# Luoyadan/CRB-active-3Ddet

Hardware: AMD Instinct MI355X
Metric: frames/s SECOND fwd+bwd, KITTI 20k-pt clouds (higher is better)
Workload: dtype f32

## Files before the change

### crb-active-3ddet_amd/crbhip/bnrelu.py

```python
import torch

from ._lib import lib, check, ptr, cur_stream, require_cuda


FUSE_RUNNING = __import__('os').environ.get('CRB_BN_FUSE_RUNNING', '1') == '1'
TICKETS = __import__('os').environ.get('CRB_BN_TICKETS', '1') == '1'
_ticket_areas = {}


def _scratch(dev, wsb):
    ws = torch.empty((wsb,), dtype=torch.uint8, device=dev)
    if not TICKETS:
        return ws, None
    key = (dev.index, torch.cuda.current_stream(dev).cuda_stream)
    t = _ticket_areas.get(key)
    if t is None:
        t = _ticket_areas[key] = torch.zeros((lib.crb_bn_ticket_ints(),), dtype=torch.int32, device=dev)
    return ws, t


def _bn_check(rc, what):
    if rc != 0:
        _ticket_areas.clear()
    check(rc, what)
# ... 216 lines not shown
@torch.no_grad()
def bn_apply_(x, bn, relu=True):
    require_cuda(x)
    n, C = x.shape
    assert x.is_contiguous()
    invstd = _invstd(bn)
    check(lib.crb_bn_relu_apply(ptr(x), n, C, ptr(bn.running_mean.contiguous()), ptr(invstd), ptr(bn.weight.contiguous()),
                                ptr(bn.bias.contiguous()), int(relu), ptr(x), 0, cur_stream(x.device)), 'crb_bn_relu_apply')
    return x


@torch.no_grad()
def bn_apply_into(x, bn, relu, out, col):
    import ctypes
    require_cuda(x, out)
    n, C = x.shape
    assert x.is_contiguous() and out.is_contiguous() and out.shape[0] == n and col + C <= out.shape[1]
    invstd = _invstd(bn)
    check(lib.crb_bn_relu_apply(ptr(x), n, C, ptr(bn.running_mean.contiguous()), ptr(invstd), ptr(bn.weight.contiguous()),
                                ptr(bn.bias.contiguous()), int(relu), ctypes.c_void_p(out.data_ptr() + 4 * col),
                                out.shape[1], cur_stream(x.device)), 'crb_bn_relu_apply')
    return out


class _BNReLUConcatTrain(torch.autograd.Function):

    @staticmethod
    def forward(ctx, relu, *args):
        import ctypes
        k = len(args) // 7
        xs = [args[7 * i].contiguous() for i in range(k)]
        n, dev = xs[0].shape[0], xs[0].device
        widths = [x.shape[1] for x in xs]
        total = sum(widths)
        out = torch.empty((n, total), dtype=torch.float32, device=dev)
        saved, col = [], 0
        for i, x in enumerate(xs):
            gamma, beta, eps, rm, rv, mom = args[7 * i + 1:7 * i + 7]
            C = widths[i]
            mean = torch.empty((C,), dtype=torch.float32, device=dev)
            var, invstd = torch.empty_like(mean), torch.empty_like(mean)
            wsb = lib.crb_bn_workspace_bytes(n, C)
            ws, tk = _scratch(dev, wsb)
            g, b = gamma.contiguous().float(), beta.contiguous().float()
            zptr = ctypes.c_void_p(out.data_ptr() + 4 * col)
            _bn_check(lib.crb_bn_relu_forward(ptr(x), n, C, ptr(g), ptr(b), float(eps), int(relu), zptr, total, ptr(mean),
                                          ptr(var), ptr(invstd), ptr(rm), ptr(rv), None, float(mom), ptr(ws), wsb, ptr(tk),
                                          cur_stream(dev)), 'crb_bn_relu_forward')
            _touch(rm, rv)
            saved += [x, mean, invstd, g, b]
            col += C
        ctx.save_for_backward(*saved)
        ctx.relu, ctx.widths = int(relu), widths
        return out

    @staticmethod
    def backward(ctx, dz):
        import ctypes
        dz = dz.contiguous().float()
        n, total = dz.shape
        saved = ctx.saved_tensors
        grads, col = [None], 0
        for i, C in enumerate(ctx.widths):
            x, mean, invstd, g, b = saved[5 * i:5 * i + 5]
            dev = x.device
            dx = torch.empty_like(x)
            dgamma = torch.empty((C,), dtype=torch.float32, device=dev)
            dbeta = torch.empty_like(dgamma)
            wsb = lib.crb_bn_workspace_bytes(n, C)
            ws, tk = _scratch(dev, wsb)
            dzp = ctypes.c_void_p(dz.data_ptr() + 4 * col)
            _bn_check(lib.crb_bn_relu_backward(ptr(x), dzp, total, n, C, ptr(mean), ptr(invstd), ptr(g), ptr(b), ctx.relu,
                                           ptr(dx), ptr(dgamma), ptr(dbeta), ptr(ws), wsb, ptr(tk), cur_stream(dev)),
                  'crb_bn_relu_backward')
            grads += [dx, dgamma, dbeta, None, None, None, None]
            col += C
        return tuple(grads)


def bn_relu_concat(xs, bns, relu=True):
    if _GROUPS is not None and _GROUPS.G > 1:
        off = _GROUPS.offsets(xs[0])
        if not torch.is_grad_enabled():
            total = sum(x.shape[1] for x in xs)
            out = torch.empty((xs[0].shape[0], total), dtype=torch.float32, device=xs[0].device)
            col = 0
            for x, bn in zip(xs, bns):
                _frames_forward(x, off, bn, relu, out, col)
                col += x.shape[1]
            return out
        with frame_groups(1):
            return torch.cat([bn_relu_concat([x[a:b] for x in xs], bns, relu) for a, b in zip(off[:-1], off[1:])], 0)
    args = []
    for x, bn in zip(xs, bns):
        with torch.no_grad():
            bn.num_batches_tracked += 1
        args += [x, bn.weight, bn.bias, bn.eps, bn.running_mean, bn.running_var, float(bn.momentum)]
    return _BNReLUConcatTrain.apply(relu, *args)


class _BNReLUMaxConcatTrain(torch.autograd.Function):

    @staticmethod
    def forward(ctx, *args):
        import ctypes
        k = len(args) // 8
        xs = [args[8 * i].contiguous() for i in range(k)]
        nss = [int(args[8 * i + 1]) for i in range(k)]
        dev = xs[0].device
        M = xs[0].shape[0] // nss[0]
        widths = [x.shape[1] for x in xs]
        total = sum(widths)
        out = torch.empty((M, total), dtype=torch.float32, device=dev)
        saved, col = [], 0
        for i, x in enumerate(xs):
            gamma, beta, eps, rm, rv, mom = args[8 * i + 2:8 * i + 8]
            C, ns = widths[i], nss[i]
            assert x.shape[0] == M * ns
            mean = torch.empty((C,), dtype=torch.float32, device=dev)
            var, invstd = torch.empty_like(mean), torch.empty_like(mean)
            arg = torch.empty((M, C), dtype=torch.int32, device=dev)
            wsb = lib.crb_bn_workspace_bytes(M * ns, C)
            ws, tk = _scratch(dev, wsb)
            g, b = gamma.contiguous().float(), beta.contiguous().float()
            zptr = ctypes.c_void_p(out.data_ptr() + 4 * col)
            _bn_check(lib.crb_bn_relu_max_forward(ptr(x), M, ns, C, ptr(g), ptr(b), float(eps), zptr, total, ptr(arg),
                                              ptr(mean), ptr(var), ptr(invstd), ptr(rm), ptr(rv), None, float(mom), ptr(ws), wsb,
                                              ptr(tk), cur_stream(dev)), 'crb_bn_relu_max_forward')
            _touch(rm, rv)
            saved += [x, mean, invstd, g, b, arg]
            col += C
        ctx.save_for_backward(*saved)
        ctx.widths, ctx.nss = widths, nss
        return out

    @staticmethod
    def backward(ctx, gz):
        import ctypes
        gz = gz.contiguous().float()
        M, total = gz.shape
        saved = ctx.saved_tensors
        grads, col = [], 0
        for i, (C, ns) in enumerate(zip(ctx.widths, ctx.nss)):
            x, mean, invstd, g, b, arg = saved[6 * i:6 * i + 6]
            dev = x.device
            dx = torch.empty_like(x)
            dgamma = torch.empty((C,), dtype=torch.float32, device=dev)
            dbeta = torch.empty_like(dgamma)
            wsb = lib.crb_bn_workspace_bytes(M * ns, C)
            ws, tk = _scratch(dev, wsb)
            gp = ctypes.c_void_p(gz.data_ptr() + 4 * col)
# ... 46 lines not shown
```

### crb-active-3ddet_amd/pcdet/models/backbones_2d/base_bev_backbone.py

```python
import numpy as np
import torch
import torch.nn as nn

from crbhip import bnrelu

from ...utils.fold_utils import fold_conv_bn
from ...utils.linear_rows import LinearRows, rows_view, rows_to_nchw


ROWS_TRAIN = True
ROWS_GEMM = True
WINOGRAD = __import__('os').environ.get('CRB_WINOGRAD', '1') != '0'


def _wino_fold(w, shift):
    from crbhip import winograd
    return winograd.weights_forward2(w), shift.contiguous()


def _wino_ok(conv, x, pad=None):
    if not WINOGRAD or not isinstance(conv, nn.Conv2d) or not x.is_cuda or x.dtype != torch.float32:
        return False
    from crbhip import winograd
    p = tuple(conv.padding) if pad is None else tuple(pad)
# ... 189 lines not shown
    def forward(self, data_dict):
        spatial_features = data_dict['spatial_features']
        ups = []
        x = spatial_features
        if not self.training and not torch.is_grad_enabled():
            cat_ok = x.is_cuda and x.is_contiguous(memory_format=torch.channels_last) and self._can_fuse_concat_eval(x)
            pre = []
            for i, blk in enumerate(self.blocks):
                x = self._run_folded(blk, x)
                if cat_ok:
                    pre.append(self._up(self.deblocks[i][0], x))
                else:
                    ups.append(self._run_folded(self.deblocks[i], x) if len(self.deblocks) > 0 else x)
            if cat_ok and all(p.is_contiguous(memory_format=torch.channels_last) and p.shape[2:] == pre[0].shape[2:]
                              for p in pre):
                n, _, h, w_ = pre[0].shape
                cat = torch.empty((n * h * w_, sum(p.shape[1] for p in pre)), dtype=torch.float32, device=x.device)
                col = 0
                for d, p in zip(self.deblocks, pre):
                    bnrelu.bn_apply_into(p.permute(0, 2, 3, 1).reshape(n * h * w_, p.shape[1]), d[1], True, cat, col)
                    col += p.shape[1]
                ups = [cat.view(n, h, w_, cat.shape[1]).permute(0, 3, 1, 2)]
            elif cat_ok:
                ups = [self._run_folded(nn.Sequential(*list(d)[1:]), p) for d, p in zip(self.deblocks, pre)]
            x = torch.cat(ups, dim=1) if len(ups) > 1 else ups[0]
            if len(self.deblocks) > len(self.blocks):
                x = self._run_folded(self.deblocks[-1], x)
            data_dict['spatial_features_2d'] = x
            return data_dict
        run = self._run_rows_train if (ROWS_TRAIN and x.is_cuda and x.is_contiguous(memory_format=torch.channels_last)) \
            else (lambda seq, t: seq(t))
        if run == self._run_rows_train and torch.is_grad_enabled():
            from crbhip import winograd
            if winograd.PREPARE:
                winograd.prepare_weights2([m.weight for blk in self.blocks for m in blk
                                           if isinstance(m, nn.Conv2d) and m.kernel_size == (3, 3) and m.stride == (1, 1)
                                           and m.weight.is_cuda])
        fuse_cat = ROWS_TRAIN and x.is_cuda and self._can_fuse_concat(x)
        pre = []
        for i, blk in enumerate(self.blocks):
            x = run(blk, x)
            stride = int(spatial_features.shape[2] / x.shape[2])
            data_dict['spatial_features_%dx' % stride] = x
            if fuse_cat:
                pre.append(self._up(self.deblocks[i][0], x))
            else:
                ups.append(run(self.deblocks[i], x) if len(self.deblocks) > 0 else x)
        if fuse_cat and all(p.is_contiguous(memory_format=torch.channels_last) and p.shape[2:] == pre[0].shape[2:]
                            for p in pre):
            n, _, h, w_ = pre[0].shape
            rows = [p.permute(0, 2, 3, 1).reshape(n * h * w_, p.shape[1]) for p in pre]
            cat = bnrelu.bn_relu_concat(rows, [d[1] for d in self.deblocks[:len(pre)]], relu=True)
            ups = [cat.view(n, h, w_, cat.shape[1]).permute(0, 3, 1, 2)]
        elif fuse_cat:
            ups = [d[2](d[1](p)) for d, p in zip(self.deblocks, pre)]
        x = torch.cat(ups, dim=1) if len(ups) > 1 else ups[0]
        if len(self.deblocks) > len(self.blocks):
            x = self.deblocks[-1](x)
        data_dict['spatial_features_2d'] = x
        if x.is_cuda:
            from crbhip import winograd
            winograd.forget_prepared_forward()
        return data_dict
```

### crb-active-3ddet_amd/pcdet/models/dense_heads/anchor_head_single.py

```python
import numpy as np
import torch
import torch.nn as nn

from ...utils.linear_rows import LinearRows, rows_view
from .anchor_head_template import AnchorHeadTemplate


FUSED_HEAD_CONVS = True
ROWS_GEMM = True


class AnchorHeadSingle(AnchorHeadTemplate):
    def __init__(self, model_cfg, input_channels, num_class, class_names, grid_size, point_cloud_range,
                 predict_boxes_when_training=True, **kwargs):
        super().__init__(model_cfg=model_cfg, num_class=num_class, class_names=class_names, grid_size=grid_size,
                         point_cloud_range=point_cloud_range, predict_boxes_when_training=predict_boxes_when_training)
        self.num_anchors_per_location = sum(self.num_anchors_per_location)
        n = self.num_anchors_per_location
        self.conv_cls = nn.Conv2d(input_channels, n * self.num_class, kernel_size=1)
        self.conv_box = nn.Conv2d(input_channels, n * self.box_coder.code_size, kernel_size=1)
        if self.model_cfg.get('USE_DIRECTION_CLASSIFIER', None) is not None:
            self.conv_dir_cls = nn.Conv2d(input_channels, n * self.model_cfg.NUM_DIR_BINS, kernel_size=1)
        else:
            self.conv_dir_cls = None
        self.lazy_box_decode = False
        self.init_weights()

    def init_weights(self):
        pi = 0.01
        nn.init.constant_(self.conv_cls.bias, -np.log((1 - pi) / pi))
        nn.init.normal_(self.conv_box.weight, mean=0, std=0.001)

    def forward(self, data_dict):
        feats = data_dict['spatial_features_2d']
        if FUSED_HEAD_CONVS:
            heads = [self.conv_cls, self.conv_box] + ([self.conv_dir_cls] if self.conv_dir_cls is not None else [])
            w = torch.cat([h.weight for h in heads], 0)
            b = torch.cat([h.bias for h in heads], 0)
            rows = rows_view(feats) if (ROWS_GEMM and feats.is_cuda) else None
            if rows is not None:
                n, _, h, w_ = feats.shape
                y = LinearRows.apply(rows, w.flatten(1), b).view(n, h, w_, w.shape[0])
            else:
                y = torch.nn.functional.conv2d(feats, w, b).permute(0, 2, 3, 1)
            outs = torch.split(y, [h.out_channels for h in heads], dim=3)
            cls_preds, box_preds = outs[0].contiguous(), outs[1].contiguous()
            dir_cls_preds = outs[2].contiguous() if self.conv_dir_cls is not None else None
        else:
            cls_preds = self.conv_cls(feats).permute(0, 2, 3, 1).contiguous()
            box_preds = self.conv_box(feats).permute(0, 2, 3, 1).contiguous()
            dir_cls_preds = None
            if self.conv_dir_cls is not None:
                dir_cls_preds = self.conv_dir_cls(feats).permute(0, 2, 3, 1).contiguous()
        self.forward_ret_dict['cls_preds'] = cls_preds
        self.forward_ret_dict['box_preds'] = box_preds
        self.forward_ret_dict['dir_cls_preds'] = dir_cls_preds
        if self.training:
            self.forward_ret_dict.update(self.assign_targets(gt_boxes=data_dict['gt_boxes']))
        if not self.training or self.predict_boxes_when_training:
            B = data_dict['batch_size']
            data_dict['rpn_preds'] = cls_preds
            data_dict['cls_preds_normalized'] = False
            if self.lazy_box_decode:
                data_dict['batch_cls_preds'] = cls_preds.view(B, -1, self.num_class).float()
                data_dict['batch_box_decoder'] = lambda idx: self.generate_predicted_boxes(
                    batch_size=B, cls_preds=cls_preds, box_preds=box_preds, dir_cls_preds=dir_cls_preds, anchor_idx=idx)[1]
                data_dict.pop('batch_box_preds', None)
            else:
                batch_cls_preds, batch_box_preds = self.generate_predicted_boxes(
                    batch_size=B, cls_preds=cls_preds, box_preds=box_preds, dir_cls_preds=dir_cls_preds)
                data_dict['batch_cls_preds'] = batch_cls_preds
                data_dict['batch_box_preds'] = batch_box_preds
        return data_dict
```

### include/crb_hip.h

```cpp
#ifndef CRB_HIP_H
#define CRB_HIP_H
#include <stdint.h>

#ifdef __cplusplus
extern "C" {
#endif

#define CRB_OK 0
#define CRB_ERR_ARG (-1)
#define CRB_ERR_WORKSPACE (-2)
#define CRB_ERR_LAUNCH (-3)
#define CRB_ERR_UNSUPPORTED (-4)

int crb_abi_version(void);

int64_t crb_voxelize_workspace_bytes(int64_t n_points, int B, int max_voxels, int max_points);
int crb_voxelize(const float* points, int64_t n_points, int num_features,
                 const int32_t* frame_offsets, int B,
                 const float* range_min_xyz, const float* voxel_size_xyz, const int32_t* grid_xyz,
                 int max_voxels, int max_points,
                 float* voxels, int32_t* coords, int32_t* num_points, float* mean_features,
                 int32_t* num_voxels_out,
                 void* workspace, int64_t workspace_bytes, void* stream);

// ... 385 lines not shown
int64_t crb_winograd2_stats_slabs(int N, int H, int W);
int crb_conv3x3_winograd2_stats_nhwc(const float* x, const float* U, float* y, float* stats, int N, int H, int W, int cin, int cout,
                                     void* stream);

int crb_winograd4_supported(int cin, int cout, int H, int W);
int64_t crb_winograd4_weights_bytes(int cin, int cout);
int crb_winograd4_weights_conv(const float* w, int64_t so, int64_t si, int64_t sky, int64_t skx, void* U, int conv_cin, int conv_cout,
                               int mode, void* stream);
int crb_winograd4_weights_conv_multi(int n, const float* const* w, const int64_t* strides, void* const* U, const int32_t* conv_cin,
                                     const int32_t* conv_cout, const int32_t* mode, void* stream);
int crb_conv3x3_winograd4_nhwc(const float* x, const void* U, float* y, int N, int H, int W, int cin, int cout, const float* bias,
                               int relu, void* stream);
int64_t crb_winograd4_stats_slabs(int N, int H, int W);
int crb_conv3x3_winograd4_stats_nhwc(const float* x, const void* U, float* y, float* stats, int N, int H, int W, int cin, int cout,
                                     void* stream);
int crb_winograd4c_supported(int cin, int cout, int H, int W);
int crb_conv3x3_winograd4c_nhwc(const float* x, const void* U, float* y, int N, int H, int W, int cin, int cout,
                                const float* bias, int relu, void* stream);
int64_t crb_winograd4c_stats_slabs(int N, int H, int W);
int crb_conv3x3_winograd4c_stats_nhwc(const float* x, const void* U, float* y, float* stats, int N, int H, int W, int cin,
                                      int cout, void* stream);

int crb_bev_blocks_geometry(int N, int H, int W, int32_t* geom);
int64_t crb_bev_blocks_ints(int N, int H, int W);
int crb_bev_blocks(const int32_t* indices, int64_t n, int N, int H, int W, int32_t* out, int64_t out_ints, void* stream);
int crb_conv3x3_winograd4c_blocks_nhwc(const float* x, const void* U, float* y, float* stats, int N, int H, int W, int cin,
                                       int cout, const int32_t* list, const int32_t* count, const int32_t* rest,
                                       const int32_t* rest_count, void* stream);

int crb_winograd2_wgrad_supported(int cin, int cout, int H, int W);
int64_t crb_winograd2_wgrad_workspace_bytes(int cin, int cout);
int crb_winograd2_wgrad(const float* x, const float* dy, float* dw, int64_t so, int64_t si, int64_t sky, int64_t skx,
                        int N, int H, int W, int cin, int cout, void* workspace, int64_t workspace_bytes, void* stream);
int crb_winograd4_wgrad_supported(int cin, int cout, int H, int W);
int64_t crb_winograd4_wgrad_workspace_bytes(int cin, int cout);
int crb_winograd4_wgrad(const float* x, const float* dy, float* dw, int64_t so, int64_t si, int64_t sky, int64_t skx,
                        int N, int H, int W, int cin, int cout, void* workspace, int64_t workspace_bytes, void* stream);
int crb_winograd4_wgrad_blocks(const float* x, const float* dy, float* dw, int64_t so, int64_t si, int64_t sky, int64_t skx,
                               int N, int H, int W, int cin, int cout, const int32_t* list, const int32_t* count,
                               void* workspace, int64_t workspace_bytes, void* stream);

int crb_rows_gemm4_supported(int cin, int cout, int stride, int direction);
int64_t crb_rows_gemm4_weights_bytes(int cin, int cout, int stride);
int crb_rows_gemm4_weights(const float* w, int64_t s_ci, int64_t s_co, int64_t s_a, int64_t s_b, void* image, int cin, int cout,
                           int stride, int direction, void* stream);
int crb_rows_gemm4_forward(const float* x, const void* image, float* y, int N, int H, int W, int cin, int cout, int stride,
                           void* stream);
int crb_rows_gemm4_input_grad(const float* dy, const void* image, float* dx, int N, int H, int W, int cin, int cout, int stride,
                              void* stream);
int64_t crb_rows_gemm4_wgrad_workspace_bytes(int cin, int cout, int stride);
int crb_rows_gemm4_wgrad(const float* x, const float* dy, float* dw, int64_t s_ci, int64_t s_co, int64_t s_a, int64_t s_b, int N,
                         int H, int W, int cin, int cout, int stride, void* workspace, int64_t workspace_bytes, void* stream);

int crb_cu_reservation(int cus, void* stream);

int crb_bev_interpolate_forward(const float* bev, int B, int H, int W, int C, const float* keypoints, int64_t M, float x_min,
                                float y_min, float voxel_x, float voxel_y, float bev_stride, float* out, void* stream);
int crb_bev_interpolate_backward(const float* dout, int B, int H, int W, int C, const float* keypoints, int64_t M, float x_min,
                                 float y_min, float voxel_x, float voxel_y, float bev_stride, float* dbev, void* stream);

int crb_roi_bev_pool(const float* bev, int B, int H, int W, int C, const float* rois, int roi_row_stride, int R, int grid_size,
                     double x_min, double y_min, double cell_x, double cell_y, float* out, void* stream);

int crb_voxel_pool_supported(int C, int nsample);
int crb_voxel_query(const float* xyz, int64_t N, const float* new_xyz, const int32_t* new_coords, int64_t M, int B,
                    const int32_t* shape_dhw, const int32_t* ranges_zyx, float radius, int nsample, const int64_t* hkeys,
                    const int32_t* hvals, int64_t capacity, int32_t* idx, int32_t* cnt, void* stream);
int64_t crb_voxel_pool_moments_workspace_bytes(int64_t M);
int crb_voxel_pool_moments(const float* xyz, const float* new_xyz, const int32_t* idx, const int32_t* cnt, int64_t M, int nsample,
                           double* sums, void* workspace, int64_t workspace_bytes, void* stream);
int crb_voxel_pool_forward(const float* features_in, int64_t N, int C, const float* xyz, const float* new_xyz, const int32_t* idx,
                           const int32_t* cnt, int64_t M, int nsample, int pool, const float* A, const float* b, float* out,
                           void* stream);
int64_t crb_voxel_pool_backward_workspace_bytes(int64_t M, int C);
int crb_voxel_pool_backward(const float* grad_out, const float* features_in, int64_t N, int C, const float* xyz,
                            const float* new_xyz, const int32_t* idx, const int32_t* cnt, int64_t M, int nsample, int pool,
                            const float* A, const float* b, float* d_features, float* g_sel, int32_t* a_row, float* d_Ab,
                            void* workspace, int64_t workspace_bytes, void* stream);

int crb_pillar_vfe_supported(int C, int T, int Cout);
int crb_pillar_vfe_num_moments(int C);
int64_t crb_pillar_vfe_moments_workspace_bytes(int64_t M, int C);
int crb_pillar_vfe_moments(const float* voxels, const int32_t* num_points, const int32_t* coords, int64_t M, int T, int C,
                           const float* voxel_size, const float* offsets, double* sums, void* workspace, int64_t workspace_bytes,
                           void* stream);
int crb_pillar_vfe_forward(const float* voxels, const int32_t* num_points, const int32_t* coords, int64_t M, int T, int C,
                           const float* voxel_size, const float* offsets, const float* A, const float* b, int Cout, float* out,
                           void* stream);
int64_t crb_pillar_vfe_backward_workspace_bytes(int64_t M, int C, int Cout);
int crb_pillar_vfe_backward(const float* grad_out, const float* voxels, const int32_t* num_points, const int32_t* coords, int64_t M,
                            int T, int C, const float* voxel_size, const float* offsets, const float* A, const float* b, int Cout,
                            double* d_sums, void* workspace, int64_t workspace_bytes, void* stream);

#define CRB_LOSSNET_MAX_LAYERS 4
typedef struct CrbLossNetArgs {
  const float* x[CRB_LOSSNET_MAX_LAYERS];
  const float* w[CRB_LOSSNET_MAX_LAYERS];
  const float* gamma[CRB_LOSSNET_MAX_LAYERS];
  const float* beta[CRB_LOSSNET_MAX_LAYERS];
  float* running_mean[CRB_LOSSNET_MAX_LAYERS];
  float* running_var[CRB_LOSSNET_MAX_LAYERS];
  int64_t* num_batches_tracked[CRB_LOSSNET_MAX_LAYERS];
  int32_t channels[CRB_LOSSNET_MAX_LAYERS];
  int32_t num_layer;
  int32_t rows_per_frame;
  int32_t frames;
// ... 110 lines not shown
```

Measured before the change: 488.9.

## Fuse head 1x1 conv backward with preceding BN-ReLU concat backward

Adds a fused backward path that joins the anchor head's 1x1 linear layer with the deblock BatchNorm+ReLU concat that feeds it. The head input gradient dz = dy·W is never materialised. A sums kernel uses split-bf16 MFMA to compute the BN reductions and dW directly from x, dy and the saved statistics, and an apply kernel recomputes dz on the fly to produce dx for both branches. This removes the full-size dz tensor, its write and reread, and a separate wgrad GEMM. The cost is a three-way bf16 split to keep f32-like accuracy, and support for only 2 branches of width 128/256 with K of 60 or 72.

```diff
diff --git a/crb-active-3ddet_amd/crbhip/bnrelu.py b/crb-active-3ddet_amd/crbhip/bnrelu.py
--- a/crb-active-3ddet_amd/crbhip/bnrelu.py
+++ b/crb-active-3ddet_amd/crbhip/bnrelu.py
@@ -292,30 +292,47 @@
             col += C
         ctx.save_for_backward(*saved)
         ctx.relu, ctx.widths = int(relu), widths
+        ctx.set_materialize_grads(False)
+        global _CONCAT_SAVED
+        _CONCAT_SAVED = saved
         return out
 
     @staticmethod
     def backward(ctx, dz):
-        import ctypes
+        if dz is None:
+            return (None,) * (1 + 7 * len(ctx.widths))
         dz = dz.contiguous().float()
-        n, total = dz.shape
         saved = ctx.saved_tensors
         grads, col = [None], 0
         for i, C in enumerate(ctx.widths):
             x, mean, invstd, g, b = saved[5 * i:5 * i + 5]
-            dev = x.device
-            dx = torch.empty_like(x)
-            dgamma = torch.empty((C,), dtype=torch.float32, device=dev)
-            dbeta = torch.empty_like(dgamma)
-            wsb = lib.crb_bn_workspace_bytes(n, C)
-            ws, tk = _scratch(dev, wsb)
-            dzp = ctypes.c_void_p(dz.data_ptr() + 4 * col)
-            _bn_check(lib.crb_bn_relu_backward(ptr(x), dzp, total, n, C, ptr(mean), ptr(invstd), ptr(g), ptr(b), ctx.relu,
-                                           ptr(dx), ptr(dgamma), ptr(dbeta), ptr(ws), wsb, ptr(tk), cur_stream(dev)),
-                  'crb_bn_relu_backward')
+            dx, dgamma, dbeta = concat_backward(x, dz, col, mean, invstd, g, b, ctx.relu)
             grads += [dx, dgamma, dbeta, None, None, None, None]
             col += C
         return tuple(grads)
+
+
+_CONCAT_SAVED = None
+
+
+def concat_backward(x, dz, col, mean, invstd, g, b, relu=1, want_dx=True):
+    import ctypes
+    n, C = x.shape
+    dev = x.device
+    dx = torch.empty_like(x) if want_dx else None
+    dgamma = torch.empty((C,), dtype=torch.float32, device=dev)
+    dbeta = torch.empty_like(dgamma)
+    wsb = lib.crb_bn_workspace_bytes(n, C)
+    ws, tk = _scratch(dev, wsb)
+    dzp = ctypes.c_void_p(dz.data_ptr() + 4 * col)
+    _bn_check(lib.crb_bn_relu_backward(ptr(x), dzp, dz.shape[1], n, C, ptr(mean), ptr(invstd), ptr(g), ptr(b), int(relu), ptr(dx),
+                                       ptr(dgamma), ptr(dbeta), ptr(ws), wsb, ptr(tk), cur_stream(dev)), 'crb_bn_relu_backward')
+    return dx, dgamma, dbeta
+
+
+def concat_reduce(x, dz, col, mean, invstd, g, b, relu=1):
+    _, dgamma, dbeta = concat_backward(x, dz, col, mean, invstd, g, b, relu, want_dx=False)
+    return dbeta, dgamma
 
 
 def bn_relu_concat(xs, bns, relu=True):
@@ -336,7 +353,14 @@
         with torch.no_grad():
             bn.num_batches_tracked += 1
         args += [x, bn.weight, bn.bias, bn.eps, bn.running_mean, bn.running_var, float(bn.momentum)]
-    return _BNReLUConcatTrain.apply(relu, *args)
+    global _CONCAT_SAVED
+    out = _BNReLUConcatTrain.apply(relu, *args)
+    saved, _CONCAT_SAVED = _CONCAT_SAVED, None
+    if torch.is_grad_enabled() and saved is not None:
+        from . import head_bn
+        out._crb_head_bn = head_bn.Record(out, [(x, bn.weight, bn.bias) for x, bn in zip(xs, bns)],
+                                          [tuple(saved[5 * i:5 * i + 5]) for i in range(len(xs))], relu)
+    return out
 
 
 class _BNReLUMaxConcatTrain(torch.autograd.Function):
diff --git a/crb-active-3ddet_amd/crbhip/head_bn.py b/crb-active-3ddet_amd/crbhip/head_bn.py
--- /dev/null
+++ b/crb-active-3ddet_amd/crbhip/head_bn.py
@@ -0,0 +1,171 @@
+import os
+
+import torch
+
+from ._lib import lib, check, ptr, cur_stream
+
+ENABLED = os.environ.get('CRB_HEAD_BN', '1') == '1'
+DEFAULT_LAUNCHES = 'sums,apply'
+LAUNCHES = set(v.strip() for v in os.environ.get('CRB_HEAD_BN_LAUNCHES', DEFAULT_LAUNCHES).split(',') if v.strip())
+
+TRACE = None
+
+
+def supported(widths, K):
+    widths = [int(v) for v in widths]
+    return len(widths) > 0 and len(set(widths)) == 1 and bool(lib.crb_head_bn_supported(len(widths), widths[0], int(K)))
+
+
+class Record(object):
+
+    def __init__(self, rows, inputs, saved, relu):
+        self.rows_ptr, self.rows_shape = rows.data_ptr(), tuple(rows.shape)
+        self.inputs = inputs
+        self.saved = saved
+        self.relu = bool(relu)
+
+    @property
+    def widths(self):
+        return [s[0].shape[1] for s in self.saved]
+
+
+def dispatch(rows, record, K):
+    if not ENABLED:
+        return 'vendor', 'CRB_HEAD_BN=0'
+    if record is None:
+        return 'vendor', 'the map carries no BatchNorm record (eval mode, grad mode off, frame_groups or another producer)'
+    if not torch.is_grad_enabled():
+        return 'vendor', 'grad mode is off'
+    if not (rows.is_cuda and rows.dim() == 2 and rows.dtype == torch.float32 and rows.is_contiguous()):
+        return 'vendor', 'the map is not a contiguous f32 device row matrix'
+    if rows.data_ptr() != record.rows_ptr or tuple(rows.shape) != record.rows_shape:
+        return 'vendor', 'the record belongs to another map'
+    if not record.relu:
+        return 'vendor', 'BatchNorm without ReLU'
+    if not supported(record.widths, K):
+        return 'vendor', 'no instance for widths %s with K = %d' % (record.widths, K)
+    return 'fused', ','.join(sorted(LAUNCHES & {'sums', 'apply'}))
+
+
+_WS = {}
+
+
+def _workspace(dev, nbytes):
+    key = (dev, torch.cuda.current_stream(dev).cuda_stream)
+    ws = _WS.get(key)
+    if ws is None or ws.numel() < nbytes:
+        ws = _WS[key] = torch.empty((nbytes,), dtype=torch.uint8, device=dev)
+    return ws
+
+
+def params(saved):
+    return torch.cat([torch.stack([s[1], s[2], s[3], s[4]]) for s in saved], 1).contiguous()
+
+
+def sums(xs, par, dout, K):
+    n, width, nb = xs[0].shape[0], xs[0].shape[1], len(xs)
+    out = torch.empty((int(lib.crb_head_bn_sums_count(nb, width, K)),), dtype=torch.float64, device=dout.device)
+    nbytes = int(lib.crb_head_bn_workspace_bytes(nb, width, K))
+    ws = _workspace(dout.device, nbytes)
+    check(lib.crb_head_bn_sums(ptr(xs[0]), ptr(xs[1]), ptr(par), ptr(dout), n, nb, width, K, ptr(out), ptr(ws), ws.numel(),
+                               cur_stream(dout.device)), 'crb_head_bn_sums')
+    return out
+
+
+def finalize(s, w, par, nb, width, K, want_bias=True):
+    Ct = nb * width
+    dgb = torch.empty((2, Ct), dtype=torch.float32, device=w.device)
+    dw = torch.empty((K, Ct), dtype=torch.float32, device=w.device)
+    db = torch.empty((K,), dtype=torch.float32, device=w.device) if want_bias else None
+    check(lib.crb_head_bn_finalize(ptr(s), ptr(w), ptr(par), nb, width, K, ptr(dgb), ptr(dw), ptr(db), cur_stream(w.device)),
+          'crb_head_bn_finalize')
+    return dgb, dw, db
+
+
+def apply(xs, par, dgb, dout, w, K):
+    n, width, nb = xs[0].shape[0], xs[0].shape[1], len(xs)
+    img = torch.empty((int(lib.crb_head_bn_weights_bytes(nb, width, K)),), dtype=torch.uint8, device=w.device)
+    check(lib.crb_head_bn_weights(ptr(w), ptr(img), nb, width, K, cur_stream(w.device)), 'crb_head_bn_weights')
+    dxs = [torch.empty_like(x) for x in xs]
+    check(lib.crb_head_bn_apply(ptr(xs[0]), ptr(xs[1]), ptr(par), ptr(dgb), ptr(dout), ptr(img), n, nb, width, K, ptr(dxs[0]),
+                                ptr(dxs[1]), cur_stream(w.device)), 'crb_head_bn_apply')
+    return dxs
+
+
+def _note(what):
+    if TRACE is not None:
+        TRACE.append(what)
+
+
+class _HeadBN(torch.autograd.Function):
+
+    @staticmethod
+    def forward(ctx, rows, w, b, record, *branch):
+        ctx.set_materialize_grads(False)
+        ctx.nb = len(record.saved)
+        ctx.launches = set(LAUNCHES)
+        flat = [t for s in record.saved for t in s]
+        ctx.save_for_backward(w, *(flat + ([rows] if 'sums' not in ctx.launches else [])))
+        return torch.addmm(b, rows, w.t())
+
+    @staticmethod
+    def backward(ctx, dy):
+        nb = ctx.nb
+        none = (None,) * (4 + 3 * nb)
+        if dy is None:
+            return none
+        t = ctx.saved_tensors
+        w = t[0].contiguous()
+        saved = [t[1 + 5 * i:6 + 5 * i] for i in range(nb)]
+        xs = [s[0] for s in saved]
+        need = ctx.needs_input_grad
+        need_x = any(need[4 + 3 * i] for i in range(nb))
+        need_gb = any(need[5 + 3 * i] or need[6 + 3 * i] for i in range(nb))
+        dy = dy.contiguous().float()
+        K, width = w.shape[0], xs[0].shape[1]
+        dw = db = dgb = None
+        dxs = [None] * nb
+        dz = None
+        if need[1] or need_gb or need_x:
+            par = params(saved)
+            if 'sums' in ctx.launches:
+                _note('sums')
+                dgb, dw, db = finalize(sums(xs, par, dy, K), w, par, nb, width, K, want_bias=need[2])
+            else:
+                from pcdet.utils.linear_rows import tall_t_matmul
+                from . import bnrelu
+                _note('vendor_sums')
+                dz = dy @ w
+                dgb = torch.empty((2, nb * width), dtype=torch.float32, device=dy.device)
+                for i, (x, mean, invstd, g, be) in enumerate(saved):
+                    dgb[:, i * width:(i + 1) * width] = torch.stack(bnrelu.concat_reduce(x, dz, i * width, mean, invstd, g, be))
+                dw = tall_t_matmul(dy, t[-1]) if need[1] else None
+            if need_x:
+                if 'apply' in ctx.launches:
+                    _note('apply')
+                    dxs = apply(xs, par, dgb, dy, w, K)
+                else:
+                    from . import bnrelu
+                    _note('vendor_apply')
+                    dz = dy @ w if dz is None else dz
+                    dxs = [bnrelu.concat_backward(x, dz, i * width, mean, invstd, g, be)[0]
+                           for i, (x, mean, invstd, g, be) in enumerate(saved)]
+        if need[2] and db is None:
+            db = dy.sum(0)
+        grads = [None, dw if need[1] else None, db if need[2] else None, None]
+        for i in range(nb):
+            sl = slice(i * width, (i + 1) * width)
+            grads += [dxs[i] if need[4 + 3 * i] else None,
+                      dgb[1, sl] if (dgb is not None and need[5 + 3 * i]) else None,
+                      dgb[0, sl] if (dgb is not None and need[6 + 3 * i]) else None]
+        return tuple(grads)
+
+
+def linear(rows, w, b, record):
+    path, _ = dispatch(rows, record, w.shape[0])
+    if path != 'fused':
+        return None
+    if b is None or w.dim() != 2 or w.dtype != torch.float32 or w.shape[1] != rows.shape[1]:
+        return None
+    branch = [t for trio in record.inputs for t in trio]
+    return _HeadBN.apply(rows, w, b, record, *branch)
diff --git a/crb-active-3ddet_amd/csrc/head_bn.hip b/crb-active-3ddet_amd/csrc/head_bn.hip
--- /dev/null
+++ b/crb-active-3ddet_amd/csrc/head_bn.hip
@@ -0,0 +1,472 @@
+#include <atomic>
+#include <type_traits>
+#include <utility>
+#include "crb_common.h"
+#include "winograd_split.h"
+#include "../../include/crb_hip.h"
+
+typedef float hb_f32x4 __attribute__((ext_vector_type(4)));
+typedef float hb_f32x16 __attribute__((ext_vector_type(16)));
+
+namespace {
+
+constexpr int HB_NT = 256;
+constexpr int HB_RBG = 8;
+constexpr int HB_COLP = 96;
+
+template <typename F, int... I>
+__device__ __forceinline__ void hb_static_for_impl(F&& f, std::integer_sequence<int, I...>) {
+  (f(std::integral_constant<int, I>{}), ...);
+}
+template <int N, typename F>
+__device__ __forceinline__ void hb_static_for(F&& f) { hb_static_for_impl(f, std::make_integer_sequence<int, N>{}); }
+
+__device__ constexpr int hb_pass_a(int p) { return p == 0 ? 0 : p == 1 ? 2 : p == 2 ? 1 : p == 3 ? 0 : p == 4 ? 1 : 0; }
+__device__ constexpr int hb_pass_b(int p) { return p == 0 ? 2 : p == 1 ? 0 : p == 2 ? 1 : p == 3 ? 1 : 0; }
+
+__device__ __forceinline__ hb_f32x16 hb_mfma(const bf16x8& a, const bf16x8& b, const hb_f32x16& c) {
+  return __builtin_amdgcn_mfma_f32_32x32x16_bf16(a, b, c, 0, 0, 0);
+}
+
+struct HbSplit8 {
+  float sv[2], s1[2], s2[2];
+  u32x4 q0, q1, q2;
+  template <int E>
+  __device__ __forceinline__ void put(float v) {
+    constexpr int hh = E & 1;
+    sv[hh] = v;
+    split3f(v, s1[hh], s2[hh]);
+    if constexpr (hh == 1) {
+      q0[E >> 1] = __builtin_amdgcn_perm(__float_as_uint(sv[1]), __float_as_uint(sv[0]), 0x07060302u);
+      q1[E >> 1] = __builtin_amdgcn_perm(__float_as_uint(s1[1]), __float_as_uint(s1[0]), 0x07060302u);
+      q2[E >> 1] = __builtin_amdgcn_perm(__float_as_uint(s2[1]), __float_as_uint(s2[0]), 0x07060302u);
+    }
+  }
+  __device__ __forceinline__ void get(bf16x8 (&f)[3]) const {
+    f[0] = __builtin_bit_cast(bf16x8, q0);
+    f[1] = __builtin_bit_cast(bf16x8, q1);
+    f[2] = __builtin_bit_cast(bf16x8, q2);
+  }
+};
+
+struct HsArgs {
+  const float* x0;
+  const float* x1;
+  const float* par;
+  const float* dout;
+  float* part;
+  double* colpart;
+  int64_t n;
+  int C, Ct, K, ncg;
+  int nchunks, nranges;
+};
+
+template <int NKB>
+__global__ __launch_bounds__(HB_NT, 2) void head_bn_sums_kernel(HsArgs a) {
+  const int lane = threadIdx.x & 63, wave = __builtin_amdgcn_readfirstlane(threadIdx.x >> 6);
+  const int r = lane & 31, h = lane >> 5;
+  const int cg = blockIdx.x % a.ncg, range = blockIdx.x / a.ncg;
+  const int cb = cg * 4 + wave, c = cb * 32 + r;
+  const int branch = (cb * 32) / a.C;
+  const float* const xbase = branch ? a.x1 : a.x0;
+  const unsigned cl = (unsigned)(c - branch * a.C);
+  const float mu = a.par[c], is = a.par[a.Ct + c], ga = a.par[2 * a.Ct + c], be = a.par[3 * a.Ct + c];
+  const int c_first = (int)((int64_t)range * a.nchunks / a.nranges);
+  const int c_end = (int)((int64_t)(range + 1) * a.nchunks / a.nranges);
+  const bool do_col = cg == 0 && wave == 0;
+
+  hb_f32x16 s2[NKB], s3[NKB];
+  double colsum[NKB];
+  bool kin[NKB];
+  unsigned kc[NKB];
+#pragma unroll
+  for (int kb = 0; kb < NKB; ++kb) {
+#pragma unroll
+    for (int i = 0; i < 16; ++i) { s2[kb][i] = 0.f; s3[kb][i] = 0.f; }
+    colsum[kb] = 0.0;
+    kin[kb] = 32 * kb + r < a.K;
+    kc[kb] = (unsigned)(kin[kb] ? 32 * kb + r : a.K - 1);
+  }
+
+  auto load = [&](int q, float (&xv)[8], float (&dv)[NKB][8]) __attribute__((always_inline)) {
+    const int64_t r0 = (int64_t)q * 16, rem = a.n - r0;
+    const unsigned last = (unsigned)(rem < 16 ? rem : 16) - 1u;
+    const float* const xq = xbase + r0 * a.C;
+    const float* const dq = a.dout + r0 * a.K;
+#pragma unroll
+    for (int j = 0; j < 8; ++j) {
+      const unsigned rj = min((unsigned)(8 * h + j), last);
+      xv[j] = xq[rj * (unsigned)a.C + cl];
+#pragma unroll
+      for (int kb = 0; kb < NKB; ++kb) dv[kb][j] = dq[rj * (unsigned)a.K + kc[kb]];
+    }
+  };
+
+  float xv[8], dv[NKB][8];
+  if (c_first < c_end) load(c_first, xv, dv);
+  for (int q = c_first; q < c_end; ++q) {
+    float xn[8], dn[NKB][8];
+    load(q + 1 < c_end ? q + 1 : q, xn, dn);
+    const int64_t left64 = a.n - ((int64_t)q * 16 + 8 * h);
+    const int left = left64 < 8 ? (int)left64 : 8;
+
+    HbSplit8 sx;
+    u32x4 mk;
+    unsigned mlo = 0;
+    hb_static_for<8>([&](auto jc) __attribute__((always_inline)) {
+      constexpr int j = decltype(jc)::value;
+      const float xh = (xv[j] - mu) * is;
+      const float z = ga * xh + be;
+      const bool m = j < left && z > 0.f;
+      sx.put<j>(m ? xh : 0.f);
+      const unsigned mb = m ? 0x3f80u : 0u;
+      if constexpr (j & 1) mk[j >> 1] = mlo | (mb << 16);
+      else mlo = mb;
+    });
+    bf16x8 X[3];
+    sx.get(X);
+    const bf16x8 Mk = __builtin_bit_cast(bf16x8, mk);
+
+    hb_static_for<NKB>([&](auto kc_) __attribute__((always_inline)) {
+      constexpr int kb = decltype(kc_)::value;
+      HbSplit8 sd;
+      float d[8];
+      hb_static_for<8>([&](auto jc) __attribute__((always_inline)) {
+        constexpr int j = decltype(jc)::value;
+        d[j] = (j < left && kin[kb]) ? dv[kb][j] : 0.f;
+        sd.put<j>(d[j]);
+      });
+      if (do_col) {
+#pragma unroll
+        for (int j = 0; j < 8; ++j) colsum[kb] += (double)d[j];
+      }
+      bf16x8 D[3];
+      sd.get(D);
+      hb_f32x16 t2, t3;
+#pragma unroll
+      for (int i = 0; i < 16; ++i) { t2[i] = 0.f; t3[i] = 0.f; }
+      t2 = hb_mfma(D[2], Mk, t2);
+      t2 = hb_mfma(D[1], Mk, t2);
+      t2 = hb_mfma(D[0], Mk, t2);
+      hb_static_for<6>([&](auto pc) __attribute__((always_inline)) {
+        constexpr int p = decltype(pc)::value;
+        t3 = hb_mfma(D[hb_pass_a(p)], X[hb_pass_b(p)], t3);
+      });
+      s2[kb] += t2;
+      s3[kb] += t3;
+    });
+#pragma unroll
+    for (int j = 0; j < 8; ++j) {
+      xv[j] = xn[j];
+#pragma unroll
+      for (int kb = 0; kb < NKB; ++kb) dv[kb][j] = dn[kb][j];
+    }
+  }
+
+  float* const p2 = a.part + ((int64_t)range * 2) * a.K * a.Ct + c;
+  float* const p3 = p2 + (int64_t)a.K * a.Ct;
+  hb_static_for<NKB>([&](auto kc_) __attribute__((always_inline)) {
+    constexpr int kb = decltype(kc_)::value;
+    hb_static_for<16>([&](auto ic) __attribute__((always_inline)) {
+      constexpr int i = decltype(ic)::value;
+      const int k = 32 * kb + (i & 3) + 8 * (i >> 2) + 4 * h;
+      if (k < a.K) {
+        p2[(int64_t)k * a.Ct] = s2[kb][i];
+        p3[(int64_t)k * a.Ct] = s3[kb][i];
+      }
+    });
+    if (do_col) a.colpart[((int64_t)range * 2 + h) * HB_COLP + 32 * kb + r] = colsum[kb];
+  });
+}
+
+__global__ __launch_bounds__(256) void head_bn_reduce_kernel(const float* __restrict__ part, const double* __restrict__ colpart,
+                                                             int nranges, int K, int Ct, double* __restrict__ sums) {
+  __shared__ double sh[8][32];
+  const int64_t per = (int64_t)2 * K * Ct;
+  const int il = threadIdx.x & 31, sl = threadIdx.x >> 5;
+  const int64_t id = (int64_t)blockIdx.x * 32 + il;
+  double s = 0.0;
+  if (id < per) {
+    for (int g = sl; g < nranges; g += 8) s += (double)part[g * per + id];
+  } else if (id < per + K) {
+    for (int g = sl; g < 2 * nranges; g += 8) s += colpart[(int64_t)g * HB_COLP + (id - per)];
+  }
+  sh[sl][il] = s;
+  __syncthreads();
+  if (sl == 0 && id < per + K) {
+    for (int k = 1; k < 8; ++k) s += sh[k][il];
+    sums[id] = s;
+  }
+}
+
+__global__ __launch_bounds__(256) void head_bn_finalize_kernel(const double* __restrict__ sums, const float* __restrict__ w,
+                                                               const float* __restrict__ par, int K, int Ct, float* __restrict__ dgb,
+                                                               float* __restrict__ dw, float* __restrict__ dbias) {
+  __shared__ double sb[8][32], sg[8][32];
+  const int cl = threadIdx.x & 31, sl = threadIdx.x >> 5;
+  const int c = blockIdx.x * 32 + cl;
+  const double ga = (double)par[2 * Ct + c], be = (double)par[3 * Ct + c];
+  double db = 0.0, dg = 0.0;
+  for (int k = sl; k < K; k += 8) {
+    const double p2 = sums[(int64_t)k * Ct + c], p3 = sums[(int64_t)(K + k) * Ct + c], wk = (double)w[(int64_t)k * Ct + c];
+    db += wk * p2;
+    dg += wk * p3;
+    dw[(int64_t)k * Ct + c] = (float)(ga * p3 + be * p2);
+  }
+  sb[sl][cl] = db;
+  sg[sl][cl] = dg;
+  __syncthreads();
+  if (sl == 0) {
+    for (int k = 1; k < 8; ++k) { db += sb[k][cl]; dg += sg[k][cl]; }
+    dgb[c] = (float)db;
+    dgb[Ct + c] = (float)dg;
+  }
+  if (dbias && blockIdx.x == 0 && (int)threadIdx.x < K) dbias[threadIdx.x] = (float)sums[(int64_t)2 * K * Ct + threadIdx.x];
+}
+
+__global__ __launch_bounds__(256) void head_bn_weights_kernel(const float* __restrict__ w, unsigned char* __restrict__ img, int K, int Ct,
+                                                              int NKS) {
+  const int id = blockIdx.x * 256 + threadIdx.x;
+  if (id >= (Ct >> 5) * NKS * 64) return;
+  const int lane = id & 63, r = lane & 31, h = lane >> 5;
+  const int ks = (id >> 6) % NKS, cb = (id >> 6) / NKS;
+  u32x4 q[3];
+  unsigned lo[3] = {0, 0, 0};
+#pragma unroll
+  for (int j = 0; j < 8; ++j) {
+    const int k = 16 * ks + 8 * h + j;
+    const float v = k < K ? w[(int64_t)k * Ct + cb * 32 + r] : 0.f;
+    unsigned p[3];
+    split3(v, p[0], p[1], p[2]);
+#pragma unroll
+    for (int i = 0; i < 3; ++i) {
+      if (j & 1) q[i][j >> 1] = lo[i] | (p[i] << 16);
+      else lo[i] = p[i];
+    }
+  }
+  unsigned char* dst = img + ((int64_t)(cb * NKS + ks) * 3) * 1024 + lane * 16;
+#pragma unroll
+  for (int i = 0; i < 3; ++i) *reinterpret_cast<u32x4*>(dst + i * 1024) = q[i];
+}
+
+struct HaArgs {
+  const float* x0;
+  const float* x1;
+  float* dx0;
+  float* dx1;
+  const float* par;
+  const float* dgb;
+  const float* dout;
+  const unsigned char* wimg;
+  int64_t n, nrb;
+  int C, Ct, K, ncg;
+  float inv_n;
+};
+
+template <int NKS>
+__global__ __launch_bounds__(HB_NT, 2) void head_bn_apply_kernel(HaArgs a) {
+  const int lane = threadIdx.x & 63, wave = __builtin_amdgcn_readfirstlane(threadIdx.x >> 6);
+  const int r = lane & 31, h = lane >> 5;
+  const int cg = blockIdx.x % a.ncg;
+  const int64_t rg = blockIdx.x / a.ncg;
+  const int cb = cg * 4 + wave, c = cb * 32 + r;
+  const int branch = (cb * 32) / a.C;
+  const float* const xbase = branch ? a.x1 : a.x0;
+  float* const obase = branch ? a.dx1 : a.dx0;
+  const unsigned cl = (unsigned)(c - branch * a.C);
+  const float mu = a.par[c], is = a.par[a.Ct + c], ga = a.par[2 * a.Ct + c], be = a.par[3 * a.Ct + c];
+  const float gis = ga * is, dbn = a.dgb[c] * a.inv_n, dgn = a.dgb[a.Ct + c] * a.inv_n;
+
+  bf16x8 W[NKS][3];
+#pragma unroll
+  for (int ks = 0; ks < NKS; ++ks)
+#pragma unroll
+    for (int p = 0; p < 3; ++p)
+      W[ks][p] = *reinterpret_cast<const bf16x8*>(a.wimg + ((int64_t)(cb * NKS + ks) * 3 + p) * 1024 + lane * 16);
+
+  const int64_t rb0 = rg * HB_RBG;
+  const int64_t rb1 = rb0 + HB_RBG < a.nrb ? rb0 + HB_RBG : a.nrb;
+  const int kl = 16 * (NKS - 1) + 8 * h;
+  const bool kok[2] = {kl + 4 <= a.K, kl + 8 <= a.K};
+  const unsigned klo[2] = {(unsigned)(kok[0] ? kl : a.K - 4), (unsigned)(kok[1] ? kl + 4 : a.K - 4)};
+  auto rows_of = [&](int64_t rb) __attribute__((always_inline)) {
+    const int64_t rem = a.n - rb * 32;
+    return (unsigned)(rem < 32 ? rem : 32);
+  };
+  auto load_d = [&](int64_t rb, hb_f32x4 (&raw)[NKS][2]) __attribute__((always_inline)) {
+    const float* const dq = a.dout + rb * 32 * a.K;
+    const unsigned ro = min((unsigned)r, rows_of(rb) - 1u) * (unsigned)a.K;
+#pragma unroll
+    for (int ks = 0; ks < NKS; ++ks)
+#pragma unroll
+      for (int q = 0; q < 2; ++q) {
+        const unsigned ko = ks == NKS - 1 ? klo[q] : (unsigned)(16 * ks + 8 * h + 4 * q);
+        raw[ks][q] = *reinterpret_cast<const hb_f32x4*>(dq + (ro + ko));
+      }
+  };
+
+  hb_f32x4 raw[NKS][2];
+  if (rb0 < rb1) load_d(rb0, raw);
+  for (int64_t rb = rb0; rb < rb1; ++rb) {
+    const unsigned rows = rows_of(rb);
+    const float* const xq = xbase + rb * 32 * a.C;
+    float* const oq = obase + rb * 32 * a.C;
+    float xv[16];
+#pragma unroll
+    for (int i = 0; i < 16; ++i) xv[i] = xq[min((unsigned)(4 * h + (i & 3) + 8 * (i >> 2)), rows - 1u) * (unsigned)a.C + cl];
+    hb_f32x4 rawn[NKS][2];
+    load_d(rb + 1 < rb1 ? rb + 1 : rb, rawn);
+
+    hb_f32x16 acc;
+#pragma unroll
+    for (int i = 0; i < 16; ++i) acc[i] = 0.f;
+    bf16x8 D0[NKS];
+    hb_static_for<NKS>([&](auto kc) __attribute__((always_inline)) {
+      constexpr int ks = decltype(kc)::value;
+      HbSplit8 sp;
+      hb_static_for<8>([&](auto ec) __attribute__((always_inline)) {
+        constexpr int e = decltype(ec)::value;
+        if constexpr (ks == NKS - 1) sp.put<e>(kok[e >> 2] ? raw[ks][e >> 2][e & 3] : 0.f);
+        else sp.put<e>(raw[ks][e >> 2][e & 3]);
+      });
+      bf16x8 D[3];
+      sp.get(D);
+      D0[ks] = D[0];
+      hb_static_for<5>([&](auto pc) __attribute__((always_inline)) {
+        constexpr int p = decltype(pc)::value;
+        acc = hb_mfma(D[hb_pass_a(p)], W[ks][hb_pass_b(p)], acc);
+      });
+    });
+    hb_static_for<NKS>([&](auto kc) __attribute__((always_inline)) {
+      constexpr int ks = decltype(kc)::value;
+      acc = hb_mfma(D0[ks], W[ks][0], acc);
+    });
+
+    auto value = [&](int i) __attribute__((always_inline)) {
+      const float xh = (xv[i] - mu) * is;
+      const float z = ga * xh + be;
+      const float d = z > 0.f ? acc[i] : 0.f;
+      return gis * (d - dbn - xh * dgn);
+    };
+    if (rows == 32) {
+#pragma unroll
+      for (int i = 0; i < 16; ++i) oq[(unsigned)(4 * h + (i & 3) + 8 * (i >> 2)) * (unsigned)a.C + cl] = value(i);
+    } else {
+#pragma unroll
+      for (int i = 0; i < 16; ++i) {
+        const unsigned ri = (unsigned)(4 * h + (i & 3) + 8 * (i >> 2));
+        if (ri < rows) oq[ri * (unsigned)a.C + cl] = value(i);
+      }
+    }
+#pragma unroll
+    for (int ks = 0; ks < NKS; ++ks) {
+      raw[ks][0] = rawn[ks][0];
+      raw[ks][1] = rawn[ks][1];
+    }
+  }
+}
+
+__host__ int hb_cu_count() {
+  static std::atomic<int> n_cu{0};
+  int n = n_cu.load(std::memory_order_relaxed);
+  if (!n) {
+    int dev = 0;
+    hipDeviceProp_t prop;
+    if (hipGetDevice(&dev) != hipSuccess || hipGetDeviceProperties(&prop, dev) != hipSuccess) return 256;
+    n = prop.multiProcessorCount > 0 ? prop.multiProcessorCount : 256;
+    n_cu.store(n, std::memory_order_relaxed);
+  }
+  return n;
+}
+
+__host__ int hb_ranges(int ncg) {
+  const int r = 2 * hb_cu_count() / ncg;
+  return r < 8 ? 8 : r;
+}
+
+__host__ int64_t hb_part_bytes(int nranges, int K, int Ct) { return crb_align_up((int64_t)nranges * 2 * K * Ct * 4, 256); }
+
+}
+
+extern "C" int crb_head_bn_supported(int nbranch, int width, int K) {
+  return (nbranch == 2 && (width == 128 || width == 256) && (K == 60 || K == 72)) ? 1 : 0;
+}
+
+extern "C" int64_t crb_head_bn_workspace_bytes(int nbranch, int width, int K) {
+  if (!crb_head_bn_supported(nbranch, width, K)) return 0;
+  const int Ct = nbranch * width, nranges = hb_ranges(Ct / 128);
+  return hb_part_bytes(nranges, K, Ct) + (int64_t)nranges * 2 * HB_COLP * 8;
+}
+
+extern "C" int64_t crb_head_bn_sums_count(int nbranch, int width, int K) {
+  if (!crb_head_bn_supported(nbranch, width, K)) return 0;
+  return (int64_t)2 * K * nbranch * width + K;
+}
+
+extern "C" int crb_head_bn_sums(const float* x0, const float* x1, const float* par, const float* dout, int64_t n, int nbranch, int width,
+                                int K, double* sums, void* workspace, int64_t workspace_bytes, void* stream) {
+  if (!crb_head_bn_supported(nbranch, width, K)) return CRB_ERR_UNSUPPORTED;
+  if (n <= 0 || n >= (1LL << 34) || !x0 || !x1 || !par || !dout || !sums) return CRB_ERR_ARG;
+  if (!workspace || workspace_bytes < crb_head_bn_workspace_bytes(nbranch, width, K)) return CRB_ERR_WORKSPACE;
+  HsArgs a;
+  a.x0 = x0; a.x1 = x1; a.par = par; a.dout = dout;
+  a.n = n; a.C = width; a.Ct = nbranch * width; a.K = K; a.ncg = a.Ct / 128;
+  a.nchunks = (int)((n + 15) / 16);
+  a.nranges = hb_ranges(a.ncg);
+  a.part = (float*)workspace;
+  a.colpart = (double*)((char*)workspace + hb_part_bytes(a.nranges, K, a.Ct));
+  const dim3 grid((unsigned)(a.nranges * a.ncg));
+  if (K > 64) hipLaunchKernelGGL(head_bn_sums_kernel<3>, grid, dim3(HB_NT), 0, (hipStream_t)stream, a);
+  else hipLaunchKernelGGL(head_bn_sums_kernel<2>, grid, dim3(HB_NT), 0, (hipStream_t)stream, a);
+  CRB_CHECK_LAUNCH();
+  const int64_t total = (int64_t)2 * K * a.Ct + K;
+  hipLaunchKernelGGL(head_bn_reduce_kernel, dim3((unsigned)crb_cdiv(total, 32)), dim3(256), 0, (hipStream_t)stream,
+                     (const float*)a.part, (const double*)a.colpart, a.nranges, K, a.Ct, sums);
+  CRB_CHECK_LAUNCH();
+  return CRB_OK;
+}
+
+extern "C" int crb_head_bn_finalize(const double* sums, const float* w, const float* par, int nbranch, int width, int K, float* dgb,
+                                    float* dw, float* dbias, void* stream) {
+  if (!crb_head_bn_supported(nbranch, width, K)) return CRB_ERR_UNSUPPORTED;
+  if (!sums || !w || !par || !dgb || !dw) return CRB_ERR_ARG;
+  const int Ct = nbranch * width;
+  hipLaunchKernelGGL(head_bn_finalize_kernel, dim3((unsigned)(Ct / 32)), dim3(256), 0, (hipStream_t)stream, sums, w, par, K, Ct, dgb, dw,
+                     dbias);
+  CRB_CHECK_LAUNCH();
+  return CRB_OK;
+}
+
+extern "C" int64_t crb_head_bn_weights_bytes(int nbranch, int width, int K) {
+  if (!crb_head_bn_supported(nbranch, width, K)) return 0;
+  return (int64_t)(nbranch * width / 32) * ((K + 15) / 16) * 3 * 1024;
+}
+
+extern "C" int crb_head_bn_weights(const float* w, void* image, int nbranch, int width, int K, void* stream) {
+  if (!crb_head_bn_supported(nbranch, width, K)) return CRB_ERR_UNSUPPORTED;
+  if (!w || !image) return CRB_ERR_ARG;
+  const int Ct = nbranch * width, NKS = (K + 15) / 16;
+  const int threads = (Ct / 32) * NKS * 64;
+  hipLaunchKernelGGL(head_bn_weights_kernel, dim3((unsigned)crb_cdiv(threads, 256)), dim3(256), 0, (hipStream_t)stream, w,
+                     (unsigned char*)image, K, Ct, NKS);
+  CRB_CHECK_LAUNCH();
+  return CRB_OK;
+}
+
+extern "C" int crb_head_bn_apply(const float* x0, const float* x1, const float* par, const float* dgb, const float* dout,
+                                 const void* image, int64_t n, int nbranch, int width, int K, float* dx0, float* dx1, void* stream) {
+  if (!crb_head_bn_supported(nbranch, width, K)) return CRB_ERR_UNSUPPORTED;
+  if (n <= 0 || n >= (1LL << 34) || !x0 || !x1 || !par || !dgb || !dout || !image || !dx0 || !dx1) return CRB_ERR_ARG;
+  HaArgs a;
+  a.x0 = x0; a.x1 = x1; a.dx0 = dx0; a.dx1 = dx1; a.par = par; a.dgb = dgb; a.dout = dout; a.wimg = (const unsigned char*)image;
+  a.n = n; a.nrb = (n + 31) / 32;
+  a.C = width; a.Ct = nbranch * width; a.K = K; a.ncg = a.Ct / 128;
+  a.inv_n = 1.0f / (float)n;
+  const int64_t groups = (a.nrb + HB_RBG - 1) / HB_RBG;
+  if (groups * a.ncg >= (1LL << 31)) return CRB_ERR_ARG;
+  const dim3 grid((unsigned)(groups * a.ncg));
+  if (K > 64) hipLaunchKernelGGL(head_bn_apply_kernel<5>, grid, dim3(HB_NT), 0, (hipStream_t)stream, a);
+  else hipLaunchKernelGGL(head_bn_apply_kernel<4>, grid, dim3(HB_NT), 0, (hipStream_t)stream, a);
+  CRB_CHECK_LAUNCH();
+  return CRB_OK;
+}
diff --git a/crb-active-3ddet_amd/pcdet/models/backbones_2d/base_bev_backbone.py b/crb-active-3ddet_amd/pcdet/models/backbones_2d/base_bev_backbone.py
--- a/crb-active-3ddet_amd/pcdet/models/backbones_2d/base_bev_backbone.py
+++ b/crb-active-3ddet_amd/pcdet/models/backbones_2d/base_bev_backbone.py
@@ -265,6 +265,8 @@
             rows = [p.permute(0, 2, 3, 1).reshape(n * h * w_, p.shape[1]) for p in pre]
             cat = bnrelu.bn_relu_concat(rows, [d[1] for d in self.deblocks[:len(pre)]], relu=True)
             ups = [cat.view(n, h, w_, cat.shape[1]).permute(0, 3, 1, 2)]
+            if len(self.deblocks) == len(self.blocks) and getattr(cat, '_crb_head_bn', None) is not None:
+                ups[0]._crb_head_bn = cat._crb_head_bn
         elif fuse_cat:
             ups = [d[2](d[1](p)) for d, p in zip(self.deblocks, pre)]
         x = torch.cat(ups, dim=1) if len(ups) > 1 else ups[0]
diff --git a/crb-active-3ddet_amd/pcdet/models/dense_heads/anchor_head_single.py b/crb-active-3ddet_amd/pcdet/models/dense_heads/anchor_head_single.py
--- a/crb-active-3ddet_amd/pcdet/models/dense_heads/anchor_head_single.py
+++ b/crb-active-3ddet_amd/pcdet/models/dense_heads/anchor_head_single.py
@@ -40,7 +40,14 @@
             rows = rows_view(feats) if (ROWS_GEMM and feats.is_cuda) else None
             if rows is not None:
                 n, _, h, w_ = feats.shape
-                y = LinearRows.apply(rows, w.flatten(1), b).view(n, h, w_, w.shape[0])
+                y = None
+                record = getattr(feats, '_crb_head_bn', None)
+                if record is not None:
+                    from crbhip import head_bn
+                    y = head_bn.linear(rows, w.flatten(1), b, record)
+                if y is None:
+                    y = LinearRows.apply(rows, w.flatten(1), b)
+                y = y.view(n, h, w_, w.shape[0])
             else:
                 y = torch.nn.functional.conv2d(feats, w, b).permute(0, 2, 3, 1)
             outs = torch.split(y, [h.out_channels for h in heads], dim=3)
diff --git a/include/crb_hip.h b/include/crb_hip.h
--- a/include/crb_hip.h
+++ b/include/crb_hip.h
@@ -461,6 +461,18 @@
 int crb_rows_gemm4_wgrad(const float* x, const float* dy, float* dw, int64_t s_ci, int64_t s_co, int64_t s_a, int64_t s_b, int N,
                          int H, int W, int cin, int cout, int stride, void* workspace, int64_t workspace_bytes, void* stream);
 
+int crb_head_bn_supported(int nbranch, int width, int K);
+int64_t crb_head_bn_workspace_bytes(int nbranch, int width, int K);
+int64_t crb_head_bn_sums_count(int nbranch, int width, int K);
+int crb_head_bn_sums(const float* x0, const float* x1, const float* par, const float* dout, int64_t n, int nbranch, int width, int K,
+                     double* sums, void* workspace, int64_t workspace_bytes, void* stream);
+int crb_head_bn_finalize(const double* sums, const float* w, const float* par, int nbranch, int width, int K, float* dgb, float* dw,
+                         float* dbias, void* stream);
+int64_t crb_head_bn_weights_bytes(int nbranch, int width, int K);
+int crb_head_bn_weights(const float* w, void* image, int nbranch, int width, int K, void* stream);
+int crb_head_bn_apply(const float* x0, const float* x1, const float* par, const float* dgb, const float* dout, const void* image,
+                      int64_t n, int nbranch, int width, int K, float* dx0, float* dx1, void* stream);
+
 int crb_cu_reservation(int cus, void* stream);
 
 int crb_bev_interpolate_forward(const float* bev, int B, int H, int W, int C, const float* keypoints, int64_t M, float x_min,
```

After: 497.5, median of 6. 1.8% higher.
